# bitsauce/Carla-ppo

Hardware: NVIDIA H100
Metric: VAE frames/sec @ batch 4096 (higher is better)
Workload: dtype f32

## Files before the change

### carla_ppo_b200/csrc/tapgemm.cuh

```cuda
#pragma once
#include "common.cuh"

namespace cpb {

constexpr int kMaxTaps = 25;

struct Tap {
    int dy, dx;
    long long src_off;
    long long w_off;
};

struct TapClass {
    int ntaps;
    int py, px;
    int Ho, Wo;
    Tap taps[kMaxTaps];
};

struct TapGemmParams {
    const float* src;
    const float* wmat;
    const float* bias;
    const float* mask;
    float* dst;
    int batch;
    int Hs, Ws;
    int src_pitch;
    long long src_img;
    int sstride;
    int C;
    int N;
    int ldw;
    int Hd, Wd;
    int dstride;
    int dst_pitch;
    long long dst_img;
    int relu;
    int check;
    int nclass;
    int ybatch;
    long long w_ystride, bias_ystride, dst_ystride;
    int ksplit;
    float* kpartial;
    long long kpartial_stride;
    const float* wk_hi;
    const float* wk_lo;
    int quad;
    int quad_cb;
    int quad_lcb;
    int cluster;
    int debug;
    int passes;
    TapClass cls[4];
};

int32_t launch_tapgemm(const TapGemmParams& p, cudaStream_t stream);
constexpr int kMaxKSplit = 8;
int tapgemm_pick_ksplit(int rows, int N, int ybatch, int K);
int32_t launch_ksplit_reduce(const TapGemmParams& p, cudaStream_t stream);
int32_t tapgemm_init();

struct TcWeightJob {
    long long src_off;
    long long dst_hi, dst_lo;
    int mode;
    int k, cb, cs;
    int N, C;
    long long count;
    int round_nearest;
    int ksplit;
};
__host__ __device__ constexpr int tc_bn(int N, bool ksplit) { return N % 128 == 0 && !ksplit ? 128 : (N % 64 == 0 ? 64 : 32); }
constexpr int kMaxTcWeightJobs = 12;
struct TcWeightTable {
    int njobs;
    long long total;
    TcWeightJob jobs[kMaxTcWeightJobs];
};
int32_t tc_tapgemm_init();
int tc_tapgemm_pick_ksplit(int K);
bool tc_tapgemm_supported(const TapGemmParams& p);
int32_t launch_tc_tapgemm(const TapGemmParams& p, cudaStream_t stream);
int32_t launch_tc_weights(const float* params, float* dst, const TcWeightTable& table, cudaStream_t stream);

}
```

### carla_ppo_b200/csrc/tc_tapgemm.cu

```cuda
#include "tapgemm.cuh"
#include "tc_common.cuh"

namespace cpb {

namespace {

using namespace tc;

template <int BN, int PASSES>
struct TcCfg {
    static constexpr int B_TILE_BYTES = BN * TBK * 4;
    static constexpr int B_IMAGES = PASSES == 3 ? 2 : 1;
    static constexpr int STAGE_BYTES = A_TILE_BYTES + B_IMAGES * B_TILE_BYTES;
    static constexpr int OUT_BYTES = TBM * BN * 4;
    static constexpr int STAGES = (224 * 1024 - OUT_BYTES) / STAGE_BYTES;
    static constexpr int SMEM_BYTES = STAGES * STAGE_BYTES + OUT_BYTES + 1024;
    static constexpr bool WIDE = BN == 128 && PASSES == 3;
    static constexpr int CONSUMER_REGS = WIDE ? 192 : 168, LOADER_REGS = WIDE ? 56 : 80, EPILOGUE_REGS = WIDE ? 72 : 80;
    static_assert(256 * CONSUMER_REGS + 128 * (LOADER_REGS + EPILOGUE_REGS) <= 512 * 128, "register file of one CTA");
};
constexpr int CHUNK_KB = 4;

constexpr int kConsumerWarps = 8;
constexpr int kLoaderWarp0 = 8;
constexpr int kLoaderWarps = 4;
constexpr int kLoaderThreads = kLoaderWarps * 32;
constexpr int kEpilogueWarp0 = 12;
constexpr int kEpilogueWarps = 4;
constexpr int kEpilogueThreads = kEpilogueWarps * 32;
constexpr int kTcThreads = 512;
constexpr int kLaunchRegs = 128;
template <int R> __device__ __forceinline__ void reg_grow() { asm volatile("setmaxnreg.inc.sync.aligned.u32 %0;" ::"n"(R)); }
template <int R> __device__ __forceinline__ void reg_shrink() { asm volatile("setmaxnreg.dec.sync.aligned.u32 %0;" ::"n"(R)); }

int g_tc_cluster = 1;
int g_tc_clusters[2][3] = {};

__device__ __forceinline__ uint32_t cluster_ctarank() { uint32_t r; asm volatile("mov.u32 %0, %%cluster_ctarank;" : "=r"(r)); return r; }
__device__ __forceinline__ uint32_t cluster_id_x() { uint32_t r; asm volatile("mov.u32 %0, %%clusterid.x;" : "=r"(r)); return r; }
__device__ __forceinline__ uint32_t cluster_count_x() { uint32_t r; asm volatile("mov.u32 %0, %%nclusterid.x;" : "=r"(r)); return r; }
__device__ __forceinline__ void cluster_sync_all() {
    asm volatile("barrier.cluster.arrive.release.aligned;" ::: "memory");
    asm volatile("barrier.cluster.wait.acquire.aligned;" ::: "memory");
}
__device__ __forceinline__ void mbar_expect_tx(uint64_t* bar, uint32_t bytes) {
    asm volatile("{\n\t.reg .b64 st;\n\tmbarrier.arrive.expect_tx.shared::cta.b64 st, [%0], %1;\n\t}" ::"r"(smem_u32(bar)), "r"(bytes) : "memory");
}
__device__ __forceinline__ void bulk_g2s(uint32_t dst, const void* src, uint32_t bytes, uint64_t* bar, uint16_t mask, bool multicast) {
    if (multicast)
        asm volatile("cp.async.bulk.shared::cluster.global.mbarrier::complete_tx::bytes.multicast::cluster [%0], [%1], %2, [%3], %4;"
                     ::"r"(dst), "l"(src), "r"(bytes), "r"(smem_u32(bar)), "h"(mask) : "memory");
    else
        asm volatile("cp.async.bulk.shared::cluster.global.mbarrier::complete_tx::bytes [%0], [%1], %2, [%3];"
                     ::"r"(dst), "l"(src), "r"(bytes), "r"(smem_u32(bar)) : "memory");
}

template <int BN, int PASSES, bool KSPLIT>
__global__ void __maxnreg__(kLaunchRegs)
tc_tapgemm_kernel(const __grid_constant__ TapGemmParams p, const int mgroups, const int total_w) {
    static_assert(PASSES == 3 || PASSES == 1, "3xTF32 or a single TF32 pass");
    using Cfg = TcCfg<BN, PASSES>;
    constexpr int STAGES = Cfg::STAGES;
    constexpr int B_TILE_BYTES = Cfg::B_TILE_BYTES;
    constexpr int STAGE_BYTES = Cfg::STAGE_BYTES;

    extern __shared__ uint8_t smem_raw[];
    __shared__ uint64_t full_bar[STAGES];
    __shared__ uint64_t empty_bar[STAGES];
    __shared__ uint64_t out_full;
    __shared__ uint64_t out_empty;

    const int tid = threadIdx.x;
    const int warp = __shfl_sync(0xffffffffu, tid >> 5, 0), lane = tid & 31;
    const int ntn = p.N / BN;
    const int CS = (int)p.cluster;
    const int rank = CS > 1 ? (int)cluster_ctarank() : 0;
    const int cl_id = CS > 1 ? (int)cluster_id_x() : (int)blockIdx.x;
    const int cl_n = CS > 1 ? (int)cluster_count_x() : (int)gridDim.x;
    const uint16_t cl_mask = (uint16_t)((1u << CS) - 1u);
    const uint32_t smem_base = (smem_u32(smem_raw) + 1023u) & ~1023u;
    const uint32_t out_base = smem_base + STAGES * STAGE_BYTES;

    if (tid == 0) {
#pragma unroll
        for (int s = 0; s < STAGES; ++s) { mbar_init(&full_bar[s], kLoaderThreads + 1); mbar_init(&empty_bar[s], (uint32_t)(kConsumerWarps * CS)); }
        mbar_init(&out_full, kConsumerWarps);
        mbar_init(&out_empty, kEpilogueWarps);
        asm volatile("fence.mbarrier_init.release.cluster;" ::: "memory");
    }
    __syncthreads();
    if (CS > 1) cluster_sync_all();

    auto st_z = [&](int st) { return st / (ntn * mgroups); };
    auto st_y = [&](int st) { return st % ntn; };
    auto st_m0 = [&](int st) { return (long long)(((st / ntn) % mgroups) * CS + rank) * TBM; };
    const int kb_per_tap = p.C / TBK;
    const int ksplit = KSPLIT ? p.ksplit : 1;
    auto split_kb = [&](int nkb, int ks) { return (int)((long long)nkb * ks / ksplit); };

    if (warp >= kEpilogueWarp0) {
        reg_shrink<Cfg::EPILOGUE_REGS>();
        constexpr int CPR = BN / 4;
        constexpr int RPP = kEpilogueThreads / CPR;
        constexpr int NR = TBM / RPP;
        constexpr uint32_t SKIP = 0xffffffffu;
        const int et = tid - kEpilogueWarp0 * 32;
        const int ec = et % CPR, er = et / CPR;
        const uint32_t o_src = out_base + (uint32_t)(er * (BN * 4) + ((ec ^ ((er & 3) << 1)) << 4));
        uint32_t phO = 0;
        for (int w = cl_id; w < total_w && !(p.debug & 16); w += cl_n) {
            const int st = KSPLIT ? w / ksplit : w, ks = KSPLIT ? w - st * ksplit : 0;
            const TapClass& cls = p.cls[st_z(st)];
            float* const dst = KSPLIT ? p.dst + (long long)ks * p.kpartial_stride : p.dst;
            const int Wo = cls.Wo, HoWo = cls.Ho * Wo;
            const uint32_t M = (uint32_t)p.batch * (uint32_t)HoWo;
            const uint32_t wo_magic = row_magic(Wo);
            const int col = st_y(st) * BN + ec * 4;
            int ch = col, qy = 0, qx = 0;
            if (p.quad) {
                const int c = col >> p.quad_lcb;
                ch = col & (p.quad_cb - 1);
                qy = c >> 1; qx = c & 1;
            }
            const uint32_t m0 = (uint32_t)st_m0(st) + (uint32_t)er;
            const int n0 = (int)(m0 / (uint32_t)HoWo);
            const int rem0 = (int)(m0 - (uint32_t)n0 * (uint32_t)HoWo);
            uint32_t m = m0;
            int n = n0, rem = rem0;
            auto next_off = [&]() {
                const int oy = row_of(rem, wo_magic);
                const int ox = rem - oy * Wo;
                const uint32_t img = (uint32_t)n * (uint32_t)p.dst_img;
                bool ok = m < M;
                uint32_t off;
                if (p.quad) {
                    const int y = oy * 2 + qy, x = ox * 2 + qx;
                    ok = ok && y < p.Hd && x < p.Wd;
                    off = img + (uint32_t)((y * p.Wd + x) * p.dst_pitch + ch);
                } else {
                    off = img + (uint32_t)(((oy * p.dstride + cls.py) * p.Wd + (ox * p.dstride + cls.px)) * p.dst_pitch + col);
                }
                m += RPP; rem += RPP;
                while (rem >= HoWo) { rem -= HoWo; ++n; }
                return ok ? off : SKIP;
            };
            uint32_t keep[NR / 8];
            if (p.mask) {
#pragma unroll 1
                for (int b = 0; b < NR / 8; ++b) {
                    uint32_t offs[8];
                    float4 mk[8];
#pragma unroll
                    for (int u = 0; u < 8; ++u) offs[u] = next_off();
#pragma unroll
                    for (int u = 0; u < 8; ++u)
                        mk[u] = offs[u] != SKIP ? __ldg(reinterpret_cast<const float4*>(p.mask + offs[u])) : make_float4(0.f, 0.f, 0.f, 0.f);
                    uint32_t bits = 0u;
#pragma unroll
                    for (int u = 0; u < 8; ++u)
                        bits |= ((mk[u].x > 0.f ? 1u : 0u) | (mk[u].y > 0.f ? 2u : 0u) | (mk[u].z > 0.f ? 4u : 0u) | (mk[u].w > 0.f ? 8u : 0u)) << (4 * u);
#pragma unroll
                    for (int q = 0; q < NR / 8 - 1; ++q) keep[q] = keep[q + 1];
                    keep[NR / 8 - 1] = bits;
                }
                m = m0; n = n0; rem = rem0;
            }
            float4 bias = make_float4(0.f, 0.f, 0.f, 0.f);
            if (p.bias) bias = __ldg(reinterpret_cast<const float4*>(p.bias + ch));

            mbar_wait(&out_full, phO);
            phO ^= 1u;
#pragma unroll 1
            for (int b = 0; b < NR / 8; ++b) {
                uint32_t offs[8];
                float4 sums[8];
#pragma unroll
                for (int u = 0; u < 8; ++u)
                    asm volatile("ld.shared.v4.f32 {%0, %1, %2, %3}, [%4];" : "=f"(sums[u].x), "=f"(sums[u].y), "=f"(sums[u].z), "=f"(sums[u].w)
                                 : "r"(o_src + (uint32_t)((8 * b + u) * RPP * BN * 4)));
#pragma unroll
                for (int u = 0; u < 8; ++u) offs[u] = next_off();
                const uint32_t bits = p.mask ? keep[0] : 0u;
#pragma unroll
                for (int q = 0; q < NR / 8 - 1; ++q) keep[q] = keep[q + 1];
#pragma unroll
                for (int u = 0; u < 8; ++u) {
                    if (offs[u] == SKIP) continue;
                    float4 o = sums[u];
                    if (p.bias) { o.x += bias.x; o.y += bias.y; o.z += bias.z; o.w += bias.w; }
                    if (p.relu) { o.x = fmaxf(o.x, 0.f); o.y = fmaxf(o.y, 0.f); o.z = fmaxf(o.z, 0.f); o.w = fmaxf(o.w, 0.f); }
                    if (p.mask) {
                        const uint32_t k = bits >> (4 * u);
                        o.x = (k & 1u) ? o.x : 0.f; o.y = (k & 2u) ? o.y : 0.f; o.z = (k & 4u) ? o.z : 0.f; o.w = (k & 8u) ? o.w : 0.f;
                    }
                    *reinterpret_cast<float4*>(dst + offs[u]) = o;
                }
            }
            __syncwarp();
            if (lane == 0) mbar_arrive(&out_empty);
        }
    } else if (warp >= kLoaderWarp0) {
        reg_shrink<Cfg::LOADER_REGS>();
        const int tl = tid - kLoaderWarp0 * 32;
        const int a_chunk = tl & 7;
        const uint32_t a_soff0 = (uint32_t)((tl >> 6) * 1024 + ((tl >> 3) & 7) * 128 + ((a_chunk ^ ((tl >> 3) & 7)) << 4));
        constexpr int RPP = kLoaderThreads / 8;
        constexpr int RPT = TBM / RPP;

        int wA = cl_id, stA = 0, tapA = 0, cA = 0;
        int kbLeftA = 0;
        int ntapsA = 0;
        int offA = 0;
        uint32_t tapbitA = 1u;
        const TapClass* clsA = &p.cls[0];
        uint32_t a_base[RPT];
        uint32_t a_taps[RPT];
        auto setup_rows = [&]() {
            stA = KSPLIT ? wA / ksplit : wA;
            const int ksA = wA - stA * ksplit;
            clsA = &p.cls[st_z(stA)];
            ntapsA = clsA->ntaps;
            const int Wo = clsA->Wo, HoWo = clsA->Ho * Wo;
            const long long M = (long long)p.batch * HoWo;
            const uint32_t wo_magic = row_magic(Wo);
            long long m = st_m0(stA) + (tl >> 3);
            int n = (int)(m / HoWo);
            int rem = (int)(m - (long long)n * HoWo);
            int iy[RPT], ix[RPT];
#pragma unroll
            for (int i = 0; i < RPT; ++i) {
                const int oy = row_of(rem, wo_magic);
                const int ox = rem - oy * Wo;
                iy[i] = oy * p.sstride; ix[i] = ox * p.sstride;
                a_base[i] = (uint32_t)n * (uint32_t)p.src_img + (uint32_t)((iy[i] * p.Ws + ix[i]) * p.src_pitch + a_chunk * 4);
                a_taps[i] = m < M ? 0xffffffffu : 0u;
                m += RPP; rem += RPP;
                while (rem >= HoWo) { rem -= HoWo; ++n; }
            }
            if (p.check) {
                uint32_t in[RPT];
#pragma unroll
                for (int i = 0; i < RPT; ++i) in[i] = 0u;
                for (int t = 0; t < ntapsA; ++t) {
                    const int dy = clsA->taps[t].dy, dx = clsA->taps[t].dx;
#pragma unroll
                    for (int i = 0; i < RPT; ++i)
                        if ((unsigned)(iy[i] + dy) < (unsigned)p.Hs && (unsigned)(ix[i] + dx) < (unsigned)p.Ws) in[i] |= 1u << t;
                }
#pragma unroll
                for (int i = 0; i < RPT; ++i) a_taps[i] &= in[i];
            }
            if constexpr (KSPLIT) {
                const int nkb = ntapsA * kb_per_tap;
                const int kb0 = split_kb(nkb, ksA);
                kbLeftA = split_kb(nkb, ksA + 1) - kb0;
                tapA = kb0 / kb_per_tap;
                cA = (kb0 - tapA * kb_per_tap) * TBK;
                offA = (int)clsA->taps[tapA].src_off + cA;
                tapbitA = 1u << tapA;
            } else {
                offA = (int)clsA->taps[0].src_off;
                tapbitA = 1u;
            }
        };
        if (wA < total_w) setup_rows();
        auto issue_a = [&](uint32_t stage, uint64_t* full) {
            const uint32_t dst = stage + a_soff0;
#pragma unroll
            for (int i = 0; i < RPT; ++i) {
                const bool v = (a_taps[i] & tapbitA) != 0u;
                const uint32_t off = v ? a_base[i] + (uint32_t)offA : 0u;
                const uint32_t bytes = (v && !(p.debug & 4)) ? 16u : 0u;
                if (p.debug & 2) continue;
                asm volatile("cp.async.cg.shared.global [%0], [%1], 16, %2;" ::"r"(dst + i * 2048), "l"(p.src + off), "r"(bytes) : "memory");
            }
            asm volatile("cp.async.mbarrier.arrive.noinc.shared::cta.b64 [%0];" ::"r"(smem_u32(full)) : "memory");
            cA += TBK; offA += TBK;
            if constexpr (KSPLIT) {
                if (--kbLeftA == 0) {
                    wA += cl_n;
                    if (wA < total_w) setup_rows();
                } else if (cA == p.C) {
                    cA = 0;
                    ++tapA;
                    offA = (int)clsA->taps[tapA].src_off;
                    tapbitA <<= 1;
                }
            } else if (cA == p.C) {
                cA = 0;
                if (++tapA == ntapsA) {
                    tapA = 0;
                    wA += cl_n;
                    if (wA < total_w) setup_rows();
                } else {
                    offA = (int)clsA->taps[tapA].src_off;
                    tapbitA <<= 1;
                }
            }
        };

        constexpr int B_BYTES = Cfg::B_IMAGES * B_TILE_BYTES;
        const uint32_t slice = (uint32_t)(B_BYTES / CS);
        auto issue_b = [&](uint32_t stage, uint64_t* full) {
            if (p.debug & 8) { mbar_arrive(full); return; }
            mbar_expect_tx(full, (uint32_t)B_BYTES);
            const float* wt = p.wk_hi + 2 * clsA->taps[tapA].w_off + ((long long)st_y(stA) * kb_per_tap + cA / TBK) * (2 * BN * TBK);
            bulk_g2s(stage + A_TILE_BYTES + (uint32_t)rank * slice, reinterpret_cast<const char*>(wt) + (size_t)rank * slice,
                     slice, full, cl_mask, CS > 1);
        };

        int sS = 0;
        uint32_t phS = 1;
        while (wA < total_w) {
            mbar_wait(&empty_bar[sS], phS);
            if (tl == 0) issue_b(smem_base + sS * STAGE_BYTES, &full_bar[sS]);
            issue_a(smem_base + sS * STAGE_BYTES, &full_bar[sS]);
            if (++sS == STAGES) { sS = 0; phS ^= 1u; }
        }
    } else {
        reg_grow<Cfg::CONSUMER_REGS>();
        constexpr int HALF = BN / 2;
        constexpr bool SACC = BN == 128;
        const int wg = warp >> 2;
        float acc[SACC ? 1 : HALF];
        float dm[HALF], dc[HALF];
#pragma unroll
        for (int i = 0; i < HALF; ++i) { dm[i] = 0.f; dc[i] = 0.f; }
        if constexpr (!SACC) {
#pragma unroll
            for (int i = 0; i < HALF; ++i) acc[i] = 0.f;
        }

        auto release = [&](int s) {
            if (lane < CS) {
                if (CS > 1) mbar_arrive_cluster(&empty_bar[s], (uint32_t)lane);
                else mbar_arrive(&empty_bar[s]);
            }
        };

        const int r0 = wg * 64 + (warp & 3) * 16 + (lane >> 2);
        const uint32_t a_row = (uint32_t)((r0 >> 3) * 1024 + (r0 & 7) * 128 + ((r0 & 7) << 4) + (lane & 3) * 4);

        const uint32_t o_dst = (uint32_t)(r0 * (BN * 4) + ((r0 & 3) << 5) + (lane & 3) * 8);
        uint32_t phE = 1;
        auto hand_off = [&]() {
            mbar_wait(&out_empty, phE);
            phE ^= 1u;
#pragma unroll
            for (int j = 0; j < BN / 8; ++j)
#pragma unroll
                for (int h = 0; h < 2; ++h)
                    asm volatile("st.shared.v2.f32 [%0], {%1, %2};" ::"r"(out_base + (uint32_t)(h * 8 * BN * 4) + (o_dst ^ (uint32_t)(j << 5))),
                                 "f"(acc[4 * j + 2 * h]), "f"(acc[4 * j + 2 * h + 1]) : "memory");
            __syncwarp();
            if (lane == 0) mbar_arrive(&out_full);
        };

        int g = 0;
        for (int w = cl_id; w < total_w; w += cl_n) {
            const int st = KSPLIT ? w / ksplit : w, ks = KSPLIT ? w - st * ksplit : 0;
            const int nkb_tile = p.cls[st_z(st)].ntaps * kb_per_tap;
            const int nkb = KSPLIT ? split_kb(nkb_tile, ks + 1) - split_kb(nkb_tile, ks) : nkb_tile;
            for (int kb = 0; kb < nkb; ++kb, ++g) {
                const int s = g % STAGES;
                const uint32_t stage = smem_base + s * STAGE_BYTES;
                mbar_wait(&full_bar[s], (uint32_t)((g / STAGES) & 1));
                uint32_t ahi[TBK / 8][4], alo[TBK / 8][4];
                uint32_t a_at = stage + a_row;
                asm volatile("" : "+r"(a_at));
#pragma unroll
                for (int ks = 0; ks < TBK / 8; ++ks)
#pragma unroll
                    for (int h = 0; h < 2; ++h)
#pragma unroll
                        for (int v = 0; v < 2; ++v) {
                            float x;
                            asm volatile("ld.shared.f32 %0, [%1];" : "=f"(x)
                                         : "r"((a_at ^ (uint32_t)((2 * ks + h) << 4)) + (uint32_t)(v * 1024)));
                            if constexpr (PASSES == 3) {
                                float hi, lo;
                                split_tf32(x, hi, lo);
                                ahi[ks][2 * h + v] = __float_as_uint(hi);
                                alo[ks][2 * h + v] = __float_as_uint(lo);
                            } else {
                                ahi[ks][2 * h + v] = round_tf32(x);
                            }
                        }
#pragma unroll
                for (int ks = 0; ks < TBK / 8; ++ks)
#pragma unroll
                    for (int i = 0; i < 4; ++i) {
                        if constexpr (PASSES == 3) asm volatile("" : "+r"(ahi[ks][i]), "+r"(alo[ks][i]));
                        else asm volatile("" : "+r"(ahi[ks][i]));
                    }
                const uint64_t b_hi = make_desc(stage + A_TILE_BYTES);
                const uint64_t b_lo = make_desc(stage + A_TILE_BYTES + B_TILE_BYTES);
                wgmma_fence();
#pragma unroll
                for (int ks = 0; ks < TBK / 8; ++ks) {
                    const uint64_t adv = (uint64_t)(ks * 2);
                    const uint32_t keep = ((kb % CHUNK_KB) | ks) != 0 ? 1u : 0u;
                    wgmma_tf32_rs<BN>(dm, ahi[ks], b_hi + adv, keep);
                    if constexpr (PASSES == 3) {
                        wgmma_tf32_rs<BN>(dc, ahi[ks], b_lo + adv, keep);
                        wgmma_tf32_rs<BN>(dc, alo[ks], b_hi + adv, 1u);
                    }
                }
                wgmma_commit();
                wgmma_wait<0>();
                fence_regs<HALF>(dm);
                if constexpr (PASSES == 3) fence_regs<HALF>(dc);
                release(s);
                if (kb % CHUNK_KB == CHUNK_KB - 1 || kb == nkb - 1) {
                    if constexpr (SACC) {
                        const bool first = kb < CHUNK_KB;
                        if (first && !(p.debug & 16)) {
                            mbar_wait(&out_empty, phE);
                            phE ^= 1u;
                        }
                        uint32_t ob = out_base + o_dst;
                        asm volatile("" : "+r"(ob));
#pragma unroll
                        for (int j0 = 0; j0 < BN / 8; j0 += 4) {
                            float sum[4][2][2];
#pragma unroll
                            for (int j = 0; j < 4; ++j)
#pragma unroll
                                for (int h = 0; h < 2; ++h) {
                                    sum[j][h][0] = 0.f; sum[j][h][1] = 0.f;
                                    if (!first)
                                        asm volatile("ld.shared.v2.f32 {%0, %1}, [%2];" : "=f"(sum[j][h][0]), "=f"(sum[j][h][1])
                                                     : "r"((ob ^ (uint32_t)((j0 + j) << 5)) + (uint32_t)(h * 8 * BN * 4)) : "memory");
                                }
#pragma unroll
                            for (int j = 0; j < 4; ++j)
#pragma unroll
                                for (int h = 0; h < 2; ++h) {
#pragma unroll
                                    for (int c = 0; c < 2; ++c) {
                                        sum[j][h][c] += dm[4 * (j0 + j) + 2 * h + c];
                                        if constexpr (PASSES == 3) sum[j][h][c] += dc[4 * (j0 + j) + 2 * h + c];
                                    }
                                    asm volatile("st.shared.v2.f32 [%0], {%1, %2};"
                                                 ::"r"((ob ^ (uint32_t)((j0 + j) << 5)) + (uint32_t)(h * 8 * BN * 4)),
                                                 "f"(sum[j][h][0]), "f"(sum[j][h][1]) : "memory");
                                }
                        }
                    } else {
#pragma unroll
                        for (int i = 0; i < HALF; ++i) {
                            acc[i] += dm[i];
                            if constexpr (PASSES == 3) acc[i] += dc[i];
                        }
                    }
                }
            }
            if constexpr (SACC) {
                if (!(p.debug & 16)) {
                    __syncwarp();
                    if (lane == 0) mbar_arrive(&out_full);
                }
            } else {
                if (!(p.debug & 16)) hand_off();
#pragma unroll
                for (int i = 0; i < HALF; ++i) acc[i] = 0.f;
            }
        }
    }
    __syncthreads();
    if (CS > 1) cluster_sync_all();
}

constexpr int tc_bn_slot(int BN) { return BN == 128 ? 2 : (BN == 64 ? 1 : 0); }
constexpr int tc_passes_slot(int PASSES) { return PASSES == 1 ? 1 : 0; }

template <int BN, int PASSES, bool KSPLIT>
int32_t tc_launch_t(const TapGemmParams& p, int mgroups, int total_w, unsigned grid, cudaStream_t stream) {
    cudaLaunchConfig_t cfg;
    memset(&cfg, 0, sizeof(cfg));
    cfg.gridDim = dim3(grid);
    cfg.blockDim = dim3(kTcThreads);
    cfg.dynamicSmemBytes = TcCfg<BN, PASSES>::SMEM_BYTES;
    cfg.stream = stream;
    cudaLaunchAttribute attr;
    attr.id = cudaLaunchAttributeClusterDimension;
    attr.val.clusterDim.x = (unsigned)p.cluster; attr.val.clusterDim.y = 1; attr.val.clusterDim.z = 1;
    cfg.attrs = &attr; cfg.numAttrs = 1;
    CPB_CUDA(cudaLaunchKernelEx(&cfg, tc_tapgemm_kernel<BN, PASSES, KSPLIT>, p, mgroups, total_w));
    CPB_LAUNCHED();
    return CPB_OK;
}

template <int BN, int PASSES>
int32_t tc_launch(const TapGemmParams& p0, cudaStream_t stream) {
    long long max_m = 0;
    for (int c = 0; c < p0.nclass; ++c) {
        long long m = (long long)p0.batch * p0.cls[c].Ho * p0.cls[c].Wo;
        if (m > max_m) max_m = m;
    }
    if (max_m == 0) return CPB_OK;
    TapGemmParams p = p0;
    p.cluster = g_tc_cluster;
    const long long mtiles = (max_m + TBM - 1) / TBM;
    const long long mgroups = (mtiles + p.cluster - 1) / p.cluster;
    const long long total_w = mgroups * (p.N / BN) * p.nclass * p.ksplit;
    const int resident = g_tc_clusters[tc_passes_slot(PASSES)][tc_bn_slot(BN)];
    CPB_REQUIRE(total_w < (1ll << 30) && resident > 0, "tc_tapgemm: bad tile count");
    CPB_REQUIRE(tc_offsets_fit(p.batch, p.src_img) && tc_offsets_fit(p.batch, p.dst_img),
                "tc_tapgemm: tensors too large for 32-bit row offsets");
    auto al16 = [](const void* q) { return (reinterpret_cast<uintptr_t>(q) & 15u) == 0; };
    CPB_REQUIRE(al16(p.dst) && al16(p.mask) && al16(p.bias) && p.dst_pitch % 4 == 0 && p.dst_img % 4 == 0 &&
                    (p.ksplit == 1 || (al16(p.kpartial) && p.kpartial_stride % 4 == 0)),
                "tc_tapgemm: destination, mask and bias must be 16-byte aligned");
    for (int c = 0; c < p.nclass; ++c) CPB_REQUIRE(p.cls[c].ntaps <= 32, "tc_tapgemm: more than 32 taps");
    if (p.quad) {
        CPB_REQUIRE((p.quad_cb & (p.quad_cb - 1)) == 0, "tc_tapgemm: quad form needs a power-of-two channel count");
        p.quad_lcb = 0;
        while ((1 << p.quad_lcb) < p.quad_cb) ++p.quad_lcb;
    }
    const unsigned grid = (unsigned)((total_w < resident ? total_w : resident) * p.cluster);
    if (p.ksplit == 1) return tc_launch_t<BN, PASSES, false>(p, (int)mgroups, (int)total_w, grid, stream);
    if constexpr (PASSES == 1 && BN <= 64) {
        TapGemmParams q = p;
        q.dst = p.kpartial; q.bias = nullptr; q.mask = nullptr; q.relu = 0;
        CPB_TRY((tc_launch_t<BN, PASSES, true>(q, (int)mgroups, (int)total_w, grid, stream)));
        return launch_ksplit_reduce(p, stream);
    } else {
        CPB_REQUIRE(false, "tc_tapgemm: the k-split is built for the single TF32 pass at BN <= 64 only");
        return CPB_ERR_UNSUPPORTED;
    }
}

template <int BN, int PASSES>
int32_t tc_init_one() {
    using Cfg = TcCfg<BN, PASSES>;
    CPB_CUDA(cudaFuncSetAttribute(tc_tapgemm_kernel<BN, PASSES, false>, cudaFuncAttributeMaxDynamicSharedMemorySize, Cfg::SMEM_BYTES));
    if (g_tc_cluster > 1) CPB_CUDA(cudaFuncSetAttribute(tc_tapgemm_kernel<BN, PASSES, false>, cudaFuncAttributeNonPortableClusterSizeAllowed, 1));
    if constexpr (PASSES == 1 && BN <= 64) {
        CPB_CUDA(cudaFuncSetAttribute(tc_tapgemm_kernel<BN, PASSES, true>, cudaFuncAttributeMaxDynamicSharedMemorySize, Cfg::SMEM_BYTES));
        if (g_tc_cluster > 1) CPB_CUDA(cudaFuncSetAttribute(tc_tapgemm_kernel<BN, PASSES, true>, cudaFuncAttributeNonPortableClusterSizeAllowed, 1));
    }
    cudaLaunchConfig_t cfg;
    memset(&cfg, 0, sizeof(cfg));
    cfg.gridDim = dim3((unsigned)(g_tc_cluster * 1024));
    cfg.blockDim = dim3(kTcThreads);
    cfg.dynamicSmemBytes = Cfg::SMEM_BYTES;
    cudaLaunchAttribute attr;
    attr.id = cudaLaunchAttributeClusterDimension;
    attr.val.clusterDim.x = (unsigned)g_tc_cluster; attr.val.clusterDim.y = 1; attr.val.clusterDim.z = 1;
    cfg.attrs = &attr; cfg.numAttrs = 1;
    int n = 0;
    CPB_CUDA(cudaOccupancyMaxActiveClusters(&n, tc_tapgemm_kernel<BN, PASSES, false>, &cfg));
    CPB_REQUIRE(n > 0, "tc_tapgemm: no resident cluster of %d CTAs possible", g_tc_cluster);
    g_tc_clusters[tc_passes_slot(PASSES)][tc_bn_slot(BN)] = n;
    return CPB_OK;
}

__global__ void tc_weights_kernel(const float* __restrict__ params, float* __restrict__ dst, const __grid_constant__ TcWeightTable t) {
    long long idx = (long long)blockIdx.x * blockDim.x + threadIdx.x;
    if (idx >= t.total) return;
    int j = 0;
    while (j < t.njobs - 1 && idx >= t.jobs[j].count) { idx -= t.jobs[j].count; ++j; }
    const TcWeightJob& job = t.jobs[j];
    float x;
    int tap, n, c;
    if (job.mode == 0) {
        tap = 0; n = (int)(idx / job.C); c = (int)(idx % job.C);
        x = params[job.src_off + idx];
    } else if (job.mode == 3) {
        tap = 0; n = (int)(idx / job.C); c = (int)(idx % job.C);
        x = params[job.src_off + (long long)c * job.N + n];
    } else if (job.mode == 2) {
        const int w = (job.k + 1) / 2;
        const int cs = (int)(idx % job.cs);
        long long rest = idx / job.cs;
        const int ncol = (int)(rest % (4 * job.cb));
        rest /= (4 * job.cb);
        const int i = (int)(rest % w), jj = (int)(rest / w);
        const int cls = ncol / job.cb, cb = ncol - cls * job.cb;
        const int kh = (cls >> 1) + 2 * jj, kw = (cls & 1) + 2 * i;
        x = (kh < job.k && kw < job.k) ? params[job.src_off + (((long long)kh * job.k + kw) * job.cb + cb) * job.cs + cs] : 0.f;
        tap = jj * w + i; n = ncol; c = cs;
    } else {
        const int run = job.k * job.cb;
        const int cc = (int)(idx % run);
        const long long rest = idx / run;
        const int cs = (int)(rest % job.cs);
        const int kh = (int)(rest / job.cs);
        const int kw = cc / job.cb, cb = cc - kw * job.cb;
        x = params[job.src_off + (((long long)kh * job.k + kw) * job.cb + cb) * job.cs + cs];
        tap = kh; n = cs; c = cc;
    }
    const int BN = tc_bn(job.N, job.ksplit != 0);
    const int nn = n % BN, cc = c % TBK;
    const long long block = ((long long)tap * (job.N / BN) + n / BN) * (job.C / TBK) + c / TBK;
    const long long at = job.dst_hi + block * (2 * BN * TBK) + (nn >> 3) * 256 + (nn & 7) * 32 + ((((cc >> 2) ^ (nn & 7))) << 2) + (cc & 3);
    const float hi = job.round_nearest ? __uint_as_float(round_tf32(x)) : __uint_as_float(__float_as_uint(x) & 0xffffe000u);
    dst[at] = hi;
    if (!job.round_nearest) dst[at + BN * TBK] = x - hi;
}

}

int32_t tc_tapgemm_init() {
    const char* e = getenv("CPB_TC_CLUSTER");
    g_tc_cluster = e ? atoi(e) : 1;
    CPB_REQUIRE(g_tc_cluster == 1 || g_tc_cluster == 2 || g_tc_cluster == 4 || g_tc_cluster == 8, "CPB_TC_CLUSTER must be 1, 2, 4 or 8");
    CPB_TRY((tc_init_one<32, 3>()));
    CPB_TRY((tc_init_one<64, 3>()));
    CPB_TRY((tc_init_one<128, 3>()));
    CPB_TRY((tc_init_one<32, 1>()));
    CPB_TRY((tc_init_one<64, 1>()));
    CPB_TRY((tc_init_one<128, 1>()));
    return CPB_OK;
}

int tc_tapgemm_pick_ksplit(int K) {
    const int s = (int)cdiv(K / TBK, 320);
    return s < 1 ? 1 : (s > 4 ? 4 : s);
}

bool tc_tapgemm_supported(const TapGemmParams& p) {
    if (p.quad && (p.N != 4 * p.quad_cb || p.nclass != 1)) return false;
    if (p.ksplit < 1 || p.ksplit > kMaxKSplit) return false;
    if (p.ksplit > 1 && (p.nclass != 1 || p.quad || p.cls[0].Ho != 1 || p.cls[0].Wo != 1 || p.dst_pitch != p.N ||
                         p.kpartial == nullptr || p.cls[0].ntaps * (p.C / TBK) < p.ksplit))
        return false;
    return p.ybatch == 1 && p.C % TBK == 0 && p.N % 32 == 0 && p.N > 0 && p.wk_hi != nullptr && p.wk_lo != nullptr;
}

int32_t launch_tc_tapgemm(const TapGemmParams& p, cudaStream_t stream) {
    CPB_REQUIRE(tc_tapgemm_supported(p), "tc_tapgemm: unsupported problem (C=%d, N=%d)", p.C, p.N);
    CPB_REQUIRE(p.passes == 3 || p.passes == 1, "tc_tapgemm: passes must be 3 or 1, got %d", p.passes);
    const int bn = tc_bn(p.N, p.ksplit > 1);
    if (p.passes == 1) return bn == 128 ? tc_launch<128, 1>(p, stream) : bn == 64 ? tc_launch<64, 1>(p, stream) : tc_launch<32, 1>(p, stream);
    return bn == 128 ? tc_launch<128, 3>(p, stream) : bn == 64 ? tc_launch<64, 3>(p, stream) : tc_launch<32, 3>(p, stream);
}

int32_t launch_tc_weights(const float* params, float* dst, const TcWeightTable& table, cudaStream_t stream) {
    if (table.total == 0) return CPB_OK;
    tc_weights_kernel<<<cdiv(table.total, 256), 256, 0, stream>>>(params, dst, table);
    CPB_LAUNCHED();
    return CPB_OK;
}

}
```

### carla_ppo_b200/csrc/vae_api.cu

```cuda
#include <algorithm>
#include <mutex>
#include <stdarg.h>

#include "elementwise.cuh"
#include "tapgemm.cuh"
#include "wgrad.cuh"

namespace cpb {

static thread_local char g_err[512] = "";
int64_t g_launches = 0;

void set_error(const char* fmt, ...) {
    va_list ap;
    va_start(ap, fmt);
    vsnprintf(g_err, sizeof(g_err), fmt, ap);
    va_end(ap);
}

bool g_profile_on = false;
namespace {
struct ProfRec { const char* label; cudaEvent_t a, b; };
constexpr int kMaxProfRecs = 4096;
ProfRec g_recs[kMaxProfRecs];
// ... 192 lines not shown
        TcW& w = r.tc[l.slot];
        w.f_hi = take(n); w.f_lo = take(n);
        w.t_hi = take(win * win * 4 * cb * cs); w.t_lo = take(win * win * 4 * cb * cs);
    }
    r.headsP = take(padded ? 2LL * FEAT * zp : 0);
    r.headsBP = take(padded ? 2LL * zp : 0);
    r.dense1P = take(padded ? (int64_t)zp * FEAT : 0);
    r.total = o;
    return r;
}

static int64_t max_partial_floats(int B, int zp, const Geo& g) {
    const int FEAT = g.FEAT;
    int64_t best = std::max<int64_t>((int64_t)edge_wgrad_ctas(B, g.frame()) * 48 * C1, (int64_t)kTcWaveCtas * 128 * 64);
    auto fit = [&](int I, int J, long long M) {
        best = std::max<int64_t>(best, (int64_t)wgrad_pick_splits(I, J, M) * I * J);
        best = std::max<int64_t>(best, (int64_t)tc_wgrad_pick_splits(I, J, M) * I * J);
    };
    fit(64, C1, (long long)B * g.s[1].H * g.s[1].W);
    for (const TcLayer& l : kTcLayers) {
        const Side &big = g.s[l.big], &small = g.s[l.small];
        fit(l.k * l.k * big.C, small.C, (long long)B * small.H * small.W);
    }
    fit(FEAT, zp, B);
    fit(zp, FEAT, B);
    return best;
}

static VaePlan make_plan(void* ws, int64_t ws_bytes, int B, int ct, int z, int mode, const Geo& g) {
    const int64_t FEAT = g.FEAT, NPIX = g.NPIX;
    const int64_t H1 = g.s[1].H, W1 = g.s[1].W, H2 = g.s[2].H, W2 = g.s[2].W, H3 = g.s[3].H, W3 = g.s[3].W;
    const int64_t C2 = g.s[2].C, C3 = g.s[3].C;
    VaePlan p;
    memset(&p, 0, sizeof(p));
    p.B = B; p.ct = ct; p.z = z; p.zp = z_pad(z); p.mode = mode; p.g = g;
    p.rl = make_relayout(z, g);
    const int64_t zp = p.zp;
    Arena a(ws, ws_bytes);
    const int64_t b = B;
    p.relayout = a.take<float>(p.rl.total);
    p.xp = a.take<float>(b * NPIX * 4);
    p.a1 = a.take<float>(b * H1 * W1 * C1);
    p.a2 = a.take<float>(b * H2 * W2 * C2);
    p.a3 = a.take<float>(b * H3 * W3 * C3);
    p.a4 = a.take<float>(b * FEAT);
    p.heads = a.take<float>(2 * b * zp);
    p.ksplit = a.take<float>((int64_t)kMaxKSplit * 2 * b * zp);
    if (mode >= CPB_WS_FORWARD) {
        p.yp = a.take<float>(b * NPIX * 4);
        p.zbuf = a.take<float>(b * zp);
        p.kl_rows = a.take<float>(b);
        p.kl_active = a.take<float>(b);
        p.frame_loss = a.take<float>(b);
        p.d1 = a.take<float>(b * FEAT);
        p.b1 = a.take<float>(b * H3 * W3 * C3);
        p.b2 = a.take<float>(b * H2 * W2 * C2);
        p.b3 = a.take<float>(b * H1 * W1 * C1);
        p.logits_p = a.take<float>(b * NPIX * 4);
    }
    if (mode >= CPB_WS_TRAIN) {
        p.gA = a.take<float>(b * H1 * W1 * C1);
        p.gB = a.take<float>(b * H1 * W1 * C1);
        p.gz = a.take<float>(b * zp);
        p.gheads = a.take<float>(2 * b * zp);
        p.partial = a.take<float>(max_partial_floats(B, p.zp, g));
        p.colsum = a.take<float>(colsum_scratch_floats(b * NPIX, 4) + colsum_scratch_floats(b * H1 * W1, C1) +
                                 colsum_scratch_floats(b, (int)FEAT));
        p.cs_edge = a.take<float>(edge_gather_blocks(B, g.frame()) * C1);
        p.frame_dsum = a.take<float>(b * 4);
    }
    p.bytes = a.off;
    return p;
}

static TapGemmParams base_params() {
    TapGemmParams p;
    memset(&p, 0, sizeof(p));
    p.nclass = 1;
    p.ybatch = 1;
    p.ksplit = 1;
    return p;
}

static TapGemmParams gather_problem(const float* big, int B, int Hb, int Wb, int pitch, int k, const float* W,
                                    int N, const float* bias, const float* mask, float* small, int relu,
                                    const float* wk_hi = nullptr, const float* wk_lo = nullptr) {
    TapGemmParams p = base_params();
    p.wk_hi = wk_hi; p.wk_lo = wk_lo;
    p.src = big; p.wmat = W; p.bias = bias; p.mask = mask; p.dst = small;
    p.batch = B; p.Hs = Hb; p.Ws = Wb; p.src_pitch = pitch; p.src_img = (long long)Hb * Wb * pitch;
    p.sstride = 2; p.C = k * pitch; p.N = N; p.ldw = N;
    const int Ho = (Hb - k) / 2 + 1, Wo = (Wb - k) / 2 + 1;
    p.Hd = Ho; p.Wd = Wo; p.dstride = 1; p.dst_pitch = N; p.dst_img = (long long)Ho * Wo * N;
    p.relu = relu; p.check = 0;
    TapClass& c = p.cls[0];
    c.ntaps = k; c.py = c.px = 0; c.Ho = Ho; c.Wo = Wo;
    for (int kh = 0; kh < k; ++kh) {
        c.taps[kh].dy = kh; c.taps[kh].dx = 0;
        c.taps[kh].src_off = (long long)kh * Wb * pitch;
        c.taps[kh].w_off = (long long)kh * k * pitch * N;
    }
    return p;
}

static TapGemmParams scatter_problem(const float* small, int B, int Hs, int Ws, int Cs, int k, const float* Wt,
                                     int Cb, const float* bias, const float* mask, float* big, int Hb, int Wb,
                                     int relu, const float* wk_hi = nullptr, const float* wk_lo = nullptr) {
    TapGemmParams p = base_params();
    p.wk_hi = wk_hi; p.wk_lo = wk_lo;
    p.src = small; p.wmat = Wt; p.bias = bias; p.mask = mask; p.dst = big;
    p.batch = B; p.Hs = Hs; p.Ws = Ws; p.src_pitch = Cs; p.src_img = (long long)Hs * Ws * Cs;
    p.sstride = 1; p.C = Cs; p.N = Cb; p.ldw = Cb;
    p.Hd = Hb; p.Wd = Wb; p.dstride = 2; p.dst_pitch = Cb; p.dst_img = (long long)Hb * Wb * Cb;
    p.relu = relu; p.check = 1; p.nclass = 4;
    for (int py = 0; py < 2; ++py)
        for (int px = 0; px < 2; ++px) {
            TapClass& c = p.cls[py * 2 + px];
            c.py = py; c.px = px;
            c.Ho = (Hb - py + 1) / 2; c.Wo = (Wb - px + 1) / 2;
            int n = 0;
            for (int kh = py, j = 0; kh < k; kh += 2, ++j)
                for (int kw = px, i = 0; kw < k; kw += 2, ++i) {
                    Tap& t = c.taps[n++];
                    t.dy = -j; t.dx = -i;
                    t.src_off = ((long long)(-j) * Ws - i) * Cs;
                    t.w_off = ((long long)kh * k + kw) * Cs * Cb;
                }
            c.ntaps = n;
        }
    return p;
}

static TapGemmParams dense_problem(const float* src, int B, int K, const float* W, int N, const float* bias,
                                   const float* mask, float* dst, int relu) {
    TapGemmParams p = base_params();
    p.src = src; p.wmat = W; p.bias = bias; p.mask = mask; p.dst = dst;
    p.batch = B; p.Hs = p.Ws = 1; p.src_pitch = K; p.src_img = K; p.sstride = 1; p.C = K; p.N = N; p.ldw = N;
    p.Hd = p.Wd = 1; p.dstride = 1; p.dst_pitch = N; p.dst_img = N; p.relu = relu; p.check = 0;
    TapClass& c = p.cls[0];
    c.ntaps = 1; c.py = c.px = 0; c.Ho = c.Wo = 1;
    c.taps[0].dy = c.taps[0].dx = 0; c.taps[0].src_off = 0; c.taps[0].w_off = 0;
    return p;
}

static TapGemmParams quad_from_scatter(const TapGemmParams& sp, int k) {
    TapGemmParams p = sp;
    const int Cb = sp.N, Cs = sp.C;
    p.quad = 1; p.quad_cb = Cb; p.N = 4 * Cb; p.nclass = 1; p.check = 1;
    TapClass& c = p.cls[0];
    const int win = (k + 1) / 2;
    c.py = c.px = 0;
    c.Ho = (sp.Hd + 1) / 2; c.Wo = (sp.Wd + 1) / 2;
    c.ntaps = win * win;
    for (int j = 0; j < win; ++j)
        for (int i = 0; i < win; ++i) {
            Tap& t = c.taps[j * win + i];
            t.dy = -j; t.dx = -i;
            t.src_off = ((long long)(-j) * sp.Ws - i) * Cs;
            t.w_off = (long long)(j * win + i) * 4 * Cb * Cs;
        }
    return p;
}

static int tc_debug_flags() {
    static const int v = [] { const char* e = getenv("CPB_TC_DEBUG"); return e ? atoi(e) : 0; }();
    return v;
}

static int32_t tg(const char* label, const TapGemmParams& p, cudaStream_t s, int scatter_k = 0) {
    ProfScope prof(label, s);
    if (g_math_mode >= 1 && p.wk_hi != nullptr) {
        TapGemmParams q = scatter_k > 0 ? quad_from_scatter(p, scatter_k) : p;
        q.debug = tc_debug_flags();
        q.passes = tc_passes();
        if (tc_tapgemm_supported(q)) return launch_tc_tapgemm(q, s);
    }
    return launch_tapgemm(p, s);
}

static int32_t run_wgrad(const TcLayer& l, const Geo& g, const float* big, const float* small, int B, float* partial, float* out,
                         cudaStream_t s) {
    ProfScope prof(l.wgrad, s);
    const Side &bs = g.s[l.big], &ss = g.s[l.small];
    WgradParams w;
    memset(&w, 0, sizeof(w));
    w.big = big; w.small = small; w.partial = partial;
    w.batch = B; w.Wb = bs.W; w.big_pitch = bs.C; w.big_img = (long long)bs.H * bs.W * bs.C;
    w.Ho = ss.H; w.Wo = ss.W; w.sstride = 2;
    w.ntaps = l.k; w.run = l.k * bs.C;
    for (int kh = 0; kh < l.k; ++kh) w.tap_off[kh] = (long long)kh * bs.W * bs.C;
    w.I = l.k * l.k * bs.C; w.J = ss.C;
    const long long M = (long long)B * ss.H * ss.W;
    if (g_math_mode >= 1 && tc_wgrad_supported(w.I, w.J, w.run)) {
        w.passes = tc_passes();
        w.splits = tc_wgrad_pick_splits(w.I, w.J, M);
        w.m_per_split = align_up((M + w.splits - 1) / w.splits, 32);
        CPB_TRY(launch_tc_wgrad(w, s));
    } else {
        w.splits = wgrad_pick_splits(w.I, w.J, M);
        w.m_per_split = align_up((M + w.splits - 1) / w.splits, 16);
        CPB_TRY(launch_wgrad(w, s));
    }
    return launch_reduce_partials(partial, w.splits, w.I, w.J, w.I, w.I, w.J, out, s);
}

static int32_t run_dense_wgrad(const char* label, const float* x, int K, int k_real, const float* g, int B, int J, int j_real,
                               float* partial, float* out, cudaStream_t s) {
    ProfScope prof(label, s);
    WgradParams w;
    memset(&w, 0, sizeof(w));
    w.big = x; w.small = g; w.partial = partial;
    w.batch = B; w.Wb = 1; w.big_pitch = K; w.big_img = K; w.Ho = w.Wo = 1; w.sstride = 1;
    w.ntaps = 1; w.run = K; w.tap_off[0] = 0; w.I = K; w.J = J;
    w.splits = wgrad_pick_splits(w.I, w.J, B);
    w.m_per_split = align_up(((long long)B + w.splits - 1) / w.splits, 16);
    CPB_TRY(launch_wgrad(w, s));
    return launch_reduce_partials(partial, w.splits, w.I, w.J, K, k_real, j_real, out, s);
}

static bool z_ok(int z) { return z >= 4 && z % 4 == 0 && z <= 1024; }
#define CPB_Z_RULE "z_dim=%d must be a multiple of 4 in [4,1024]"

static int32_t check_cfg(const cpb_vae_config* cfg) {
    CPB_REQUIRE(cfg != nullptr, "cfg is NULL");
    CPB_REQUIRE(cfg->batch >= 1 && cfg->batch <= (1 << 20), "batch=%d out of range", cfg->batch);
    CPB_REQUIRE(cfg->target_channels == 1 || cfg->target_channels == 3, "target_channels must be 1 or 3, got %d", cfg->target_channels);
    CPB_REQUIRE(z_ok(cfg->z_dim), CPB_Z_RULE, cfg->z_dim);
    CPB_REQUIRE(cfg->loss_type >= 0 && cfg->loss_type <= 2, "unknown loss_type %d", cfg->loss_type);
    CPB_REQUIRE(cfg->source_dtype == CPB_FRAME_F32 || cfg->source_dtype == CPB_FRAME_U8, "bad source_dtype");
    CPB_REQUIRE(cfg->target_dtype == CPB_FRAME_F32 || cfg->target_dtype == CPB_FRAME_U8, "bad target_dtype");
    return CPB_OK;
}

static int32_t check_frame(int H, int W) {
    CPB_REQUIRE(frame_side_ok(H) && frame_side_ok(W), CPB_FRAME_RULE, H, W);
    return CPB_OK;
}

static int32_t check_spec(const cpb_vae_spec* sp) {
    CPB_REQUIRE(sp != nullptr, "cfg is NULL");
    CPB_TRY(check_cfg(&sp->base));
    return check_frame(sp->height, sp->width);
}

static int32_t check_batch_bound(const cpb_vae_spec* sp, const Geo& g) {
    const int64_t limit = tc_batch_limit(g);
    if (g_math_mode == 0 || sp->base.batch <= limit) return CPB_OK;
    set_error("batch=%d is above %lld, the largest batch the tensor-core kernels (math modes 1 and 2) take at frame %dx%d",
              sp->base.batch, (long long)limit, sp->height, sp->width);
    return CPB_ERR_UNSUPPORTED;
}

static void add_relayout(RelayoutTable& t, int64_t src, int64_t dst, int taps, int rows, int cols, int mode,
                         int rows_pad, int cols_pad) {
    RelayoutJob& j = t.jobs[t.njobs++];
    j.src_off = src; j.dst_off = dst; j.taps = taps; j.rows = rows; j.cols = cols; j.mode = mode;
    j.rows_pad = rows_pad; j.cols_pad = cols_pad;
    j.count = (long long)taps * rows_pad * cols_pad;
    t.total += j.count;
}

struct Latent {
    int B, K, z, zp;
    const int64_t* off;
    int mean;
};

static TapGemmParams heads_fwd_problem(const Latent& h, const float* params, const float* x, const float* wp, const float* bp,
                                       float* heads) {
    const bool padded = h.zp != h.z;
    TapGemmParams p = dense_problem(x, h.B, h.K, padded ? wp : params + h.off[h.mean], h.zp,
                                    padded ? bp : params + h.off[h.mean + 1], nullptr, heads, 0);
    p.ybatch = 2;
    p.w_ystride = padded ? (long long)h.K * h.zp : h.off[h.mean + 2] - h.off[h.mean];
    p.bias_ystride = padded ? h.zp : h.off[h.mean + 3] - h.off[h.mean + 1];
    p.dst_ystride = (long long)h.B * h.zp;
    return p;
}

static int32_t heads_backward(const Latent& h, const char* wgrad_label, const char* dgrad_label, const float* x, const float* gheads,
                              const float* wt, float* gx, float* partial, float* cs, float* grads, cudaStream_t s) {
    const long long glogvar = (long long)h.B * h.zp;
    CPB_TRY(run_dense_wgrad(wgrad_label, x, h.K, h.K, gheads, h.B, h.zp, h.z, partial, grads + h.off[h.mean], s));
    CPB_TRY(run_dense_wgrad(wgrad_label, x, h.K, h.K, gheads + glogvar, h.B, h.zp, h.z, partial, grads + h.off[h.mean + 2], s));
    CPB_TRY(launch_colsum(gheads, h.B, h.zp, h.z, grads + h.off[h.mean + 1], cs, s));
    CPB_TRY(launch_colsum(gheads + glogvar, h.B, h.zp, h.z, grads + h.off[h.mean + 3], cs, s));
    TapGemmParams p = dense_problem(gheads, h.B, h.zp, wt, h.K, nullptr, x, gx, 0);
    p.cls[0].ntaps = 2;
    p.cls[0].taps[1].dy = p.cls[0].taps[1].dx = 0;
    p.cls[0].taps[1].src_off = glogvar;
    p.cls[0].taps[1].w_off = (long long)h.zp * h.K;
    if (dgrad_label == nullptr) return launch_tapgemm(p, s);
    ProfScope prof(dgrad_label, s);
    return launch_tapgemm(p, s);
}

static void add_z_padding(RelayoutTable& t, const Latent& h, bool heads, int64_t wp, int64_t bp, bool dec, int64_t dec_off,
                          int N, int64_t dp) {
    if (h.zp == h.z) return;
    if (heads) {
        add_relayout(t, h.off[h.mean], wp, 2, h.K, h.z, 1, h.K, h.zp);
        add_relayout(t, h.off[h.mean + 1], bp, 1, 1, h.z, 1, 1, h.zp);
        add_relayout(t, h.off[h.mean + 3], bp + h.zp, 1, 1, h.z, 1, 1, h.zp);
    }
    if (dec) add_relayout(t, dec_off, dp, 1, h.z, N, 1, h.zp, N);
}

static bool target_is_source(const cpb_vae_config* c, const void* source, const void* target) {
    return target == source && c->target_channels == 3 && c->target_dtype == c->source_dtype &&
           (c->target_dtype == CPB_FRAME_F32 || c->target_u8_scale == 1.f / 255.f);
}

// ... 1191 lines not shown
```

Measured before the change: 86440.

## Skip structurally-zero weight columns in quad transposed-conv TC GEMM taps

For the quad (sub-pixel) form of a transposed convolution with odd kernel size, some taps have weight columns that are all zero for certain output phases. The change reorders the phase columns so those zero columns sit together, records a per-tap dead mask, and issues narrower wgmma instructions (N=64 or 32) over a shifted B descriptor for those taps. It adds a new template variant with more epilogue branching and accumulator resets, plus host checks that dead patterns are uniform within a chunk.

Result: no change. 87010, median of 6 (+0.7%).

```diff
diff --git a/carla_ppo_b200/csrc/tapgemm.cuh b/carla_ppo_b200/csrc/tapgemm.cuh
--- a/carla_ppo_b200/csrc/tapgemm.cuh
+++ b/carla_ppo_b200/csrc/tapgemm.cuh
@@ -49,6 +49,7 @@
     int quad;
     int quad_cb;
     int quad_lcb;
+    unsigned long long quad_dead;
     int cluster;
     int debug;
     int passes;
@@ -60,6 +61,9 @@
 int tapgemm_pick_ksplit(int rows, int N, int ybatch, int K);
 int32_t launch_ksplit_reduce(const TapGemmParams& p, cudaStream_t stream);
 int32_t tapgemm_init();
+
+__host__ __device__ constexpr int quad_py(int s) { return (0x9 >> s) & 1; }
+__host__ __device__ constexpr int quad_px(int s) { return s >> 1; }
 
 struct TcWeightJob {
     long long src_off;
diff --git a/carla_ppo_b200/csrc/tc_tapgemm.cu b/carla_ppo_b200/csrc/tc_tapgemm.cu
--- a/carla_ppo_b200/csrc/tc_tapgemm.cu
+++ b/carla_ppo_b200/csrc/tc_tapgemm.cu
@@ -1,3 +1,5 @@
+#include <type_traits>
+
 #include "tapgemm.cuh"
 #include "tc_common.cuh"
 
@@ -55,10 +57,11 @@
                      ::"r"(dst), "l"(src), "r"(bytes), "r"(smem_u32(bar)) : "memory");
 }
 
-template <int BN, int PASSES, bool KSPLIT>
+template <int BN, int PASSES, bool KSPLIT, bool QDEAD>
 __global__ void __maxnreg__(kLaunchRegs)
 tc_tapgemm_kernel(const __grid_constant__ TapGemmParams p, const int mgroups, const int total_w) {
     static_assert(PASSES == 3 || PASSES == 1, "3xTF32 or a single TF32 pass");
+    static_assert(!QDEAD || (BN == 128 && PASSES == 3 && !KSPLIT), "zero taps are skipped by the 3-pass kernel at BN 128");
     using Cfg = TcCfg<BN, PASSES>;
     constexpr int STAGES = Cfg::STAGES;
     constexpr int B_TILE_BYTES = Cfg::B_TILE_BYTES;
@@ -118,9 +121,9 @@
             const int col = st_y(st) * BN + ec * 4;
             int ch = col, qy = 0, qx = 0;
             if (p.quad) {
-                const int c = col >> p.quad_lcb;
+                const int s = col >> p.quad_lcb;
                 ch = col & (p.quad_cb - 1);
-                qy = c >> 1; qx = c & 1;
+                qy = quad_py(s); qx = quad_px(s);
             }
             const uint32_t m0 = (uint32_t)st_m0(st) + (uint32_t)er;
             const int n0 = (int)(m0 / (uint32_t)HoWo);
@@ -361,6 +364,8 @@
             const int st = KSPLIT ? w / ksplit : w, ks = KSPLIT ? w - st * ksplit : 0;
             const int nkb_tile = p.cls[st_z(st)].ntaps * kb_per_tap;
             const int nkb = KSPLIT ? split_kb(nkb_tile, ks + 1) - split_kb(nkb_tile, ks) : nkb_tile;
+            unsigned long long dead_q = p.quad_dead;
+            int kt = 0;
             for (int kb = 0; kb < nkb; ++kb, ++g) {
                 const int s = g % STAGES;
                 const uint32_t stage = smem_base + s * STAGE_BYTES;
@@ -393,20 +398,36 @@
                         if constexpr (PASSES == 3) asm volatile("" : "+r"(ahi[ks][i]), "+r"(alo[ks][i]));
                         else asm volatile("" : "+r"(ahi[ks][i]));
                     }
-                const uint64_t b_hi = make_desc(stage + A_TILE_BYTES);
-                const uint64_t b_lo = make_desc(stage + A_TILE_BYTES + B_TILE_BYTES);
-                wgmma_fence();
-#pragma unroll
-                for (int ks = 0; ks < TBK / 8; ++ks) {
-                    const uint64_t adv = (uint64_t)(ks * 2);
-                    const uint32_t keep = ((kb % CHUNK_KB) | ks) != 0 ? 1u : 0u;
-                    wgmma_tf32_rs<BN>(dm, ahi[ks], b_hi + adv, keep);
-                    if constexpr (PASSES == 3) {
-                        wgmma_tf32_rs<BN>(dc, ahi[ks], b_lo + adv, keep);
-                        wgmma_tf32_rs<BN>(dc, alo[ks], b_hi + adv, 1u);
+                const bool chunk0 = kb % CHUNK_KB == 0;
+                uint32_t cshift = 0u;
+                auto mma = [&](auto nw) {
+                    constexpr int NW = decltype(nw)::value;
+                    const uint32_t b_at = stage + A_TILE_BYTES + cshift * (32u * 128u);
+                    const uint64_t b_hi = make_desc(b_at);
+                    const uint64_t b_lo = make_desc(b_at + B_TILE_BYTES);
+                    wgmma_fence();
+#pragma unroll
+                    for (int ks = 0; ks < TBK / 8; ++ks) {
+                        const uint64_t adv = (uint64_t)(ks * 2);
+                        const uint32_t keep = (!chunk0 || ks != 0) ? 1u : 0u;
+                        wgmma_tf32_rs<NW>(dm, ahi[ks], b_hi + adv, keep);
+                        if constexpr (PASSES == 3) {
+                            wgmma_tf32_rs<NW>(dc, ahi[ks], b_lo + adv, keep);
+                            wgmma_tf32_rs<NW>(dc, alo[ks], b_hi + adv, 1u);
+                        }
                     }
-                }
-                wgmma_commit();
+                    wgmma_commit();
+                };
+                if constexpr (QDEAD) {
+                    const uint32_t dead = (uint32_t)dead_q & 3u;
+                    cshift = dead >> 1;
+                    if (dead == 0u) mma(std::integral_constant<int, 128>{});
+                    else if (dead == 3u) mma(std::integral_constant<int, 32>{});
+                    else mma(std::integral_constant<int, 64>{});
+                    if (++kt == kb_per_tap) { kt = 0; dead_q >>= 2; }
+                } else {
+                    mma(std::integral_constant<int, BN>{});
+                }
                 wgmma_wait<0>();
                 fence_regs<HALF>(dm);
                 if constexpr (PASSES == 3) fence_regs<HALF>(dc);
@@ -422,6 +443,8 @@
                         asm volatile("" : "+r"(ob));
 #pragma unroll
                         for (int j0 = 0; j0 < BN / 8; j0 += 4) {
+                            if (j0 == BN / 8 - 4 && cshift != 0u) continue;
+                            const uint32_t obj = ob ^ (((uint32_t)j0 + 4u * cshift) << 5);
                             float sum[4][2][2];
 #pragma unroll
                             for (int j = 0; j < 4; ++j)
@@ -430,7 +453,7 @@
                                     sum[j][h][0] = 0.f; sum[j][h][1] = 0.f;
                                     if (!first)
                                         asm volatile("ld.shared.v2.f32 {%0, %1}, [%2];" : "=f"(sum[j][h][0]), "=f"(sum[j][h][1])
-                                                     : "r"((ob ^ (uint32_t)((j0 + j) << 5)) + (uint32_t)(h * 8 * BN * 4)) : "memory");
+                                                     : "r"((obj ^ (uint32_t)(j << 5)) + (uint32_t)(h * 8 * BN * 4)) : "memory");
                                 }
 #pragma unroll
                             for (int j = 0; j < 4; ++j)
@@ -442,7 +465,7 @@
                                         if constexpr (PASSES == 3) sum[j][h][c] += dc[4 * (j0 + j) + 2 * h + c];
                                     }
                                     asm volatile("st.shared.v2.f32 [%0], {%1, %2};"
-                                                 ::"r"((ob ^ (uint32_t)((j0 + j) << 5)) + (uint32_t)(h * 8 * BN * 4)),
+                                                 ::"r"((obj ^ (uint32_t)(j << 5)) + (uint32_t)(h * 8 * BN * 4)),
                                                  "f"(sum[j][h][0]), "f"(sum[j][h][1]) : "memory");
                                 }
                         }
@@ -454,6 +477,14 @@
                         }
                     }
                 }
+                if constexpr (QDEAD) {
+                    if ((kb + 1) % CHUNK_KB == 0 && (dead_q & 3u) != 0u) {
+#pragma unroll
+                        for (int i = 0; i < HALF; ++i) { dm[i] = 0.f; dc[i] = 0.f; }
+                        fence_regs<HALF>(dm);
+                        if constexpr (PASSES == 3) fence_regs<HALF>(dc);
+                    }
+                }
             }
             if constexpr (SACC) {
                 if (!(p.debug & 16)) {
@@ -474,7 +505,7 @@
 constexpr int tc_bn_slot(int BN) { return BN == 128 ? 2 : (BN == 64 ? 1 : 0); }
 constexpr int tc_passes_slot(int PASSES) { return PASSES == 1 ? 1 : 0; }
 
-template <int BN, int PASSES, bool KSPLIT>
+template <int BN, int PASSES, bool KSPLIT, bool QDEAD = false>
 int32_t tc_launch_t(const TapGemmParams& p, int mgroups, int total_w, unsigned grid, cudaStream_t stream) {
     cudaLaunchConfig_t cfg;
     memset(&cfg, 0, sizeof(cfg));
@@ -486,7 +517,7 @@
     attr.id = cudaLaunchAttributeClusterDimension;
     attr.val.clusterDim.x = (unsigned)p.cluster; attr.val.clusterDim.y = 1; attr.val.clusterDim.z = 1;
     cfg.attrs = &attr; cfg.numAttrs = 1;
-    CPB_CUDA(cudaLaunchKernelEx(&cfg, tc_tapgemm_kernel<BN, PASSES, KSPLIT>, p, mgroups, total_w));
+    CPB_CUDA(cudaLaunchKernelEx(&cfg, tc_tapgemm_kernel<BN, PASSES, KSPLIT, QDEAD>, p, mgroups, total_w));
     CPB_LAUNCHED();
     return CPB_OK;
 }
@@ -518,7 +549,18 @@
         p.quad_lcb = 0;
         while ((1 << p.quad_lcb) < p.quad_cb) ++p.quad_lcb;
     }
+    if (p.quad_dead != 0) {
+        CPB_REQUIRE(p.quad && BN == 128 && p.N == 128, "tc_tapgemm: zero taps are skipped at quad_cb = 32 only");
+        const int kbpt = p.C / TBK, nkb = p.cls[0].ntaps * kbpt;
+        auto shifted = [&](int kb) { return (p.quad_dead >> (2 * (kb / kbpt) + 1)) & 1u; };
+        for (int kb = 0; kb < nkb; ++kb)
+            CPB_REQUIRE(shifted(kb) == shifted(kb - kb % CHUNK_KB) && (kb >= CHUNK_KB || !shifted(kb)),
+                        "tc_tapgemm: zero taps of different shapes in one chunk");
+    }
     const unsigned grid = (unsigned)((total_w < resident ? total_w : resident) * p.cluster);
+    if constexpr (BN == 128 && PASSES == 3) {
+        if (p.quad_dead != 0) return tc_launch_t<BN, PASSES, false, true>(p, (int)mgroups, (int)total_w, grid, stream);
+    }
     if (p.ksplit == 1) return tc_launch_t<BN, PASSES, false>(p, (int)mgroups, (int)total_w, grid, stream);
     if constexpr (PASSES == 1 && BN <= 64) {
         TapGemmParams q = p;
@@ -534,11 +576,15 @@
 template <int BN, int PASSES>
 int32_t tc_init_one() {
     using Cfg = TcCfg<BN, PASSES>;
-    CPB_CUDA(cudaFuncSetAttribute(tc_tapgemm_kernel<BN, PASSES, false>, cudaFuncAttributeMaxDynamicSharedMemorySize, Cfg::SMEM_BYTES));
-    if (g_tc_cluster > 1) CPB_CUDA(cudaFuncSetAttribute(tc_tapgemm_kernel<BN, PASSES, false>, cudaFuncAttributeNonPortableClusterSizeAllowed, 1));
+    CPB_CUDA(cudaFuncSetAttribute(tc_tapgemm_kernel<BN, PASSES, false, false>, cudaFuncAttributeMaxDynamicSharedMemorySize, Cfg::SMEM_BYTES));
+    if (g_tc_cluster > 1) CPB_CUDA(cudaFuncSetAttribute(tc_tapgemm_kernel<BN, PASSES, false, false>, cudaFuncAttributeNonPortableClusterSizeAllowed, 1));
     if constexpr (PASSES == 1 && BN <= 64) {
-        CPB_CUDA(cudaFuncSetAttribute(tc_tapgemm_kernel<BN, PASSES, true>, cudaFuncAttributeMaxDynamicSharedMemorySize, Cfg::SMEM_BYTES));
-        if (g_tc_cluster > 1) CPB_CUDA(cudaFuncSetAttribute(tc_tapgemm_kernel<BN, PASSES, true>, cudaFuncAttributeNonPortableClusterSizeAllowed, 1));
+        CPB_CUDA(cudaFuncSetAttribute(tc_tapgemm_kernel<BN, PASSES, true, false>, cudaFuncAttributeMaxDynamicSharedMemorySize, Cfg::SMEM_BYTES));
+        if (g_tc_cluster > 1) CPB_CUDA(cudaFuncSetAttribute(tc_tapgemm_kernel<BN, PASSES, true, false>, cudaFuncAttributeNonPortableClusterSizeAllowed, 1));
+    }
+    if constexpr (BN == 128 && PASSES == 3) {
+        CPB_CUDA(cudaFuncSetAttribute(tc_tapgemm_kernel<BN, PASSES, false, true>, cudaFuncAttributeMaxDynamicSharedMemorySize, Cfg::SMEM_BYTES));
+        if (g_tc_cluster > 1) CPB_CUDA(cudaFuncSetAttribute(tc_tapgemm_kernel<BN, PASSES, false, true>, cudaFuncAttributeNonPortableClusterSizeAllowed, 1));
     }
     cudaLaunchConfig_t cfg;
     memset(&cfg, 0, sizeof(cfg));
@@ -550,7 +596,7 @@
     attr.val.clusterDim.x = (unsigned)g_tc_cluster; attr.val.clusterDim.y = 1; attr.val.clusterDim.z = 1;
     cfg.attrs = &attr; cfg.numAttrs = 1;
     int n = 0;
-    CPB_CUDA(cudaOccupancyMaxActiveClusters(&n, tc_tapgemm_kernel<BN, PASSES, false>, &cfg));
+    CPB_CUDA(cudaOccupancyMaxActiveClusters(&n, tc_tapgemm_kernel<BN, PASSES, false, false>, &cfg));
     CPB_REQUIRE(n > 0, "tc_tapgemm: no resident cluster of %d CTAs possible", g_tc_cluster);
     g_tc_clusters[tc_passes_slot(PASSES)][tc_bn_slot(BN)] = n;
     return CPB_OK;
@@ -577,8 +623,8 @@
         const int ncol = (int)(rest % (4 * job.cb));
         rest /= (4 * job.cb);
         const int i = (int)(rest % w), jj = (int)(rest / w);
-        const int cls = ncol / job.cb, cb = ncol - cls * job.cb;
-        const int kh = (cls >> 1) + 2 * jj, kw = (cls & 1) + 2 * i;
+        const int s = ncol / job.cb, cb = ncol - s * job.cb;
+        const int kh = quad_py(s) + 2 * jj, kw = quad_px(s) + 2 * i;
         x = (kh < job.k && kw < job.k) ? params[job.src_off + (((long long)kh * job.k + kw) * job.cb + cb) * job.cs + cs] : 0.f;
         tap = jj * w + i; n = ncol; c = cs;
     } else {
diff --git a/carla_ppo_b200/csrc/vae_api.cu b/carla_ppo_b200/csrc/vae_api.cu
--- a/carla_ppo_b200/csrc/vae_api.cu
+++ b/carla_ppo_b200/csrc/vae_api.cu
@@ -368,12 +368,15 @@
     c.py = c.px = 0;
     c.Ho = (sp.Hd + 1) / 2; c.Wo = (sp.Wd + 1) / 2;
     c.ntaps = win * win;
+    p.quad_dead = 0;
     for (int j = 0; j < win; ++j)
         for (int i = 0; i < win; ++i) {
             Tap& t = c.taps[j * win + i];
             t.dy = -j; t.dx = -i;
             t.src_off = ((long long)(-j) * sp.Ws - i) * Cs;
             t.w_off = (long long)(j * win + i) * 4 * Cb * Cs;
+            const unsigned long long dead = (2 * i + 1 >= k ? 1u : 0u) | (2 * j + 1 >= k ? 2u : 0u);
+            p.quad_dead |= dead << (2 * (j * win + i));
         }
     return p;
 }
```
